# daac-tools/daachorse

Measured on AMD Instinct MI355X. Metric: haystack GB/s scanned (find_overlapping_iter(..).count(), 100k-pattern bytewise automaton), higher is better.
Workload: dtype u8/u32 integer

## Files before the change

### daachorse_amd/csrc/device_tables.hpp

```cpp
#pragma once

#include <hip/hip_runtime.h>

#include <cstdint>

#include "../../include/daachorse_amd.h"
#include "gram4_mph.hpp"

namespace daac {

struct TierDev {
    const void *rows;
    const uint32_t *bcmap;
    const uint32_t *bfail;
    const uint2 *ssum;
    const uint8_t *cls;
    const uint4 *grec;
    const uint32_t *sopos;
    const uint32_t *outputs;
    const uint32_t *ohash;
    uint32_t C, NA, NB, N;
    uint32_t off_bcmap, off_bfail, off_ssum, off_cls, lds_bytes;
    uint32_t row32, root_flag;
};

struct DArrayDev {
    const uint2 *hot;
    const uint32_t *fail;
    const uint32_t *fail_plain;
    const uint4 *rec;
    const uint4 *root_chain;
    const uint4 *root;
    const uint2 *osum;
    const uint32_t *outputs;
    const uint32_t *ohash;
    uint32_t n, root_flag, leftmost;
};

struct CharDev {
    const uint4 *states;
    const uint32_t *fail_plain;
    const uint32_t *table;
    const uint2 *osum;
    const uint32_t *outputs;
    const uint32_t *ohash;
    uint32_t table_len, n, root_flag, leftmost;
    uint32_t map_in_lds;
    uint32_t map_lo;
    const uint2 *root_row;
    uint32_t alphabet;
    uint32_t row_in_lds;
    const uint4 *wstates;
    uint32_t obits, fbits;
};

struct ScanArgs {
    const uint8_t *hay;
    uint64_t begin;
    uint64_t len;
    uint64_t seg_bytes;
    uint64_t nseg;
    uint32_t halo;
    unsigned long long *result;
    unsigned long long *seg_counts;
    daac_match *out;
    uint64_t total_len;
    unsigned long long *flags;
};

struct ScanArgs;
struct ChainArgs;

struct ChainArgs {
    const unsigned long long *x_spec;
    const unsigned long long *x_prev;
    unsigned long long *x_out;
    unsigned int *flags;
    uint4 *tally_spec;
    uint4 *tally_delta;
    uint64_t cap;
};

struct GramDev {
    const uint32_t *cls32;
    const uint16_t *cid;
    const uint2 *combo;
    const uint32_t *bbits;
    const uint8_t *brank;
    const uint32_t *bsuper;
    const uint4 *drec;
    const uint2 *dhit;
    const uint4 *dhit4;
    const uint32_t *cfirst;
    uint32_t off_cid, off_combo, off_bbits, off_brank, off_bsuper, off_scratch, lds_bytes;
    uint32_t K, C, CC, CCC;
    uint32_t level_start, unused_byte, has_short;
    uint32_t rank_in_lds;
    uint32_t n_deep;
};

struct GramArgs {
    const uint8_t *hay_al;
    uint32_t lead;
    uint64_t vlen;
    uint64_t region_bytes;
    uint64_t nregions;
    unsigned long long *result;
    uint2 *wq;
    uint32_t wq_slab;
    uint32_t ppl;
    uint32_t dense;
    const uint32_t *sel;
    uint32_t sel_want;
};

hipError_t launch_gram_scan(const GramDev &dev, const GramArgs &a, uint32_t blocks, uint32_t threads, hipStream_t stream);

constexpr uint32_t kGram2OffH = 512;
struct Gram2Dev {
    const uint8_t *cls;
    const uint32_t *m;
    const void *sdir;
    const uint16_t *rfull;
    const uint16_t *cid4;
    const uint32_t *hsum;
    const uint4 *drec;
    const uint2 *dhit;
    const uint4 *dhit4;
    const uint32_t *cfirst;
    uint32_t m_bytes, s_bytes, cid_bytes, h_bytes;
    uint32_t off_m_count, off_s_count, off_ring_count, lds_count;
    uint32_t rfull_bytes, off_ring_rfull, lds_rfull, rfull_ok;
    uint32_t off_m_exact, off_s_exact, off_cid, off_ring_exact, lds_exact;
    uint32_t K, C, s16, unused_byte, n_deep, exact_ok;
    uint32_t xlane_dpp;
};
uint32_t gram2_lds_bytes(const Gram2Dev &dev, bool exact);

struct Gram2WDev {
    const uint8_t *cls;
    const unsigned long long *m;
    const uint32_t *sdir;
    const uint16_t *cid4;
    const uint32_t *hsum;
    const uint4 *drec;
    const uint4 *dhit;
    uint32_t m_bytes, s_bytes, cid_bytes, h_bytes;
    uint32_t off_m_count, off_s_count, off_ring_count, lds_count;
    uint32_t off_m_exact, off_s_exact, off_cid, off_ring_exact, lds_exact;
    uint32_t C, unused_byte, n_deep, exact_ok;
};
hipError_t launch_gram2w_scan(const Gram2WDev &dev, const GramArgs &a, bool exact, uint32_t blocks, hipStream_t stream);

constexpr uint32_t kGram2OffM = 512;
struct Gram2EmitDev {
    const uint8_t *cls;
    const uint32_t *me;
    const void *sdir;
    const uint32_t *v1, *v2;
    const uint32_t *v3;
    const uint4 *erec;
    const uint2 *ehit;
    const uint4 *ehit4;
    const uint32_t *dupo, *dupv;
    uint32_t level_start;
    const uint32_t *cfirst;
    uint32_t m_bytes, s_bytes, v1_bytes, v2_bytes;
    uint32_t off_s, off_v1, off_v2, off_ring, off_wave, lds_bytes;
    uint32_t K, C, s16, unused_byte;
    const uint32_t *v3c;
    uint32_t v3c_bytes, v3c_dir, v3c_val;
};
hipError_t launch_gram2_scan(const Gram2Dev &dev, const GramArgs &a, bool exact, uint32_t blocks, uint32_t threads, hipStream_t stream);

struct Gram3Lds {
    uint32_t off_s;
    uint32_t off_wave;
    uint32_t wave_stride;
    uint32_t lds_bytes, threads, rfull;
};

constexpr uint32_t kGram4EndsBitDev = 30;
struct Gram4Dev {
    const uint8_t *cls;
    const uint32_t *m;
    const uint16_t *rfull;
    const void *sdir;
    const uint2 *dhit_c;
    const uint4 *dhit_t;
    const uint4 *drec_c;
    const uint4 *drec_t;
    const uint32_t *bloom;
    uint32_t bloom_words;
    const uint8_t *mph_disp;
    const uint2 *dhit_h;
    G4Mph mph;
    uint32_t mph_bytes;
    uint32_t m_bytes, rfull_bytes, s_bytes;
    uint32_t K, C, s16, arith, lo, unused_byte, n_deep;
};
struct Gram4Lds {
    uint32_t off_wave;
    uint32_t wave_stride;
    uint32_t off_cls;
    uint32_t off_s;
    uint32_t off_m;
    uint32_t s_bytes;
    uint32_t lds_bytes, threads;
    uint32_t arith;
    uint32_t dir;
    uint32_t filter;
    uint32_t off_b;
    uint32_t s_bytes_f;
    uint32_t mph;
};
uint32_t gram4_filter_room(uint32_t m_bytes, uint32_t sdir_bytes, bool arith, uint32_t lds_limit);
bool gram4_plan(const Gram4Dev &dev, uint32_t ppl, uint32_t waves, bool rfull, bool want_arith, bool want_filter, uint32_t lds_limit, Gram4Lds &L);
hipError_t launch_gram4_scan(const Gram4Dev &dev, const GramArgs &a, const Gram4Lds &L, uint32_t blocks, hipStream_t stream);

constexpr uint32_t kEmit3Tile = 1024;
constexpr uint32_t kEmit3Chunk = 1024;
constexpr uint32_t kEmit3MaxExtrasAtPosition = 15;
constexpr uint32_t kEmit3MaxExtras = 64;
constexpr uint32_t kEmit3Stage = 960;
constexpr uint32_t kEmit3ExpandWave = (kEmit3Stage + 64) * 8 + 2048 + 256 + 1024 + kEmit3MaxExtras * 16 + 16;
constexpr uint32_t kEmit3ExpandWave16 = (kEmit3Stage + 64) * 2 + 1040 + 2048 + 256 + 1024 + kEmit3MaxExtras * 16 + 16;
struct Emit3Args {
    const uint8_t *hay_al;
    uint32_t lead;
    uint32_t vlen;
    uint32_t emit_from;
    uint8_t *ann;
    uint32_t *tile_short;
    uint32_t *tile_deep;
    uint32_t tile0;
    uint4 *recs;
    uint32_t *chunk_fill;
    uint32_t *chunk_next;
    uint32_t chunk_cap;
    uint2 *wq;
    uint32_t wq_slab;
    uint32_t region_bytes;
    uint32_t nregions;
    unsigned int *fail;
};
struct Expand3Args {
    const uint8_t *ann;
    uint32_t ntiles;
    const unsigned long long *tile_off;
    const unsigned long long *bin_off;
    const uint4 *binned;
    void *out;
    unsigned long long pos_base;
    uint32_t off_wave;
    uint32_t has_len1;
    uint32_t v3_in_lds;
    unsigned int *fail;
    uint32_t vlen, emit_from;
};
bool emit3_plan(const Gram2EmitDev &dev, uint32_t waves, uint32_t lds_limit, Gram3Lds &L);
hipError_t launch_emit3_detect(const Gram2EmitDev &dev, const Emit3Args &a, const Gram3Lds &L, uint32_t blocks, hipStream_t stream);
hipError_t launch_emit3_combine(const uint32_t *tile_short, const uint32_t *tile_deep, unsigned long long *total, unsigned long long *deep, uint64_t n,
                                hipStream_t stream);
hipError_t launch_emit3_bin(const uint4 *recs, const uint32_t *chunk_fill, const uint32_t *chunk_next, uint32_t chunk_cap, const unsigned long long *bin_off,
                            uint32_t *cursor, uint4 *binned, uint32_t n1k, unsigned long long rec_limit, uint32_t blocks, hipStream_t stream);
hipError_t launch_emit3_expand(const Gram2EmitDev &dev, const Expand3Args &a, bool f16, uint32_t blocks, hipStream_t stream);
hipError_t launch_emit3_expand_raw(const Gram2EmitDev &dev, const Expand3Args &a, bool f16, uint32_t blocks, hipStream_t stream);
uint32_t emit3_expand_lds_bytes(const Gram2EmitDev &dev, uint32_t waves, bool f16, bool v3_in_lds);

constexpr uint32_t kFind3Tile = 2048;
constexpr uint32_t kFind3Deep = 255;
constexpr uint32_t kLeft3Wave = 2080 + 4096 + 1024 + 256 + 288;
constexpr uint32_t kFind3Wave = 2064 + 4096 + 1024 + 256;
struct Find3Dev {
    const uint32_t *h1, *h2;
    const uint32_t *h3c;
    uint32_t h1_bytes, h2_bytes, h3c_bytes, h3c_dir, h3c_val, C;
};
struct Find3Args {
    const uint8_t *ann;
    uint32_t ntiles;
    uint32_t n1k;
    const unsigned long long *bin_off;
    const uint4 *binned;
    const uint32_t *entry_in;
    uint32_t *exit_out;
    uint32_t force_pos;
    unsigned long long pos_base;
    uint32_t off_wave;
    uint32_t count_only;
    unsigned long long *result;
    unsigned long long *tile_cnt;
    const unsigned long long *tile_off;
    void *out;
    uint32_t f16;
    uint32_t first_start;
    uint32_t last_start;
    uint32_t *last_sel;
    unsigned int *flag;
    const uint32_t *ctl;
    uint32_t chunk_cap;
    unsigned long long rec_limit;
};
__device__ __forceinline__ bool find3_detect_usable(const Find3Args &a) {
    return a.ctl[0] <= a.chunk_cap && a.ctl[1] == 0u && a.bin_off[a.n1k] <= a.rec_limit;
}
uint32_t find3_lds_bytes(const Find3Dev &dev, bool tally);
hipError_t launch_find3_select(const Find3Dev &dev, const Find3Args &a, bool has_len1, bool tally, uint32_t blocks, hipStream_t stream);
hipError_t launch_find3_emit(const Find3Dev &dev, const Find3Args &a, bool has_len1, uint32_t blocks, hipStream_t stream);
hipError_t launch_left3_emit(const Find3Dev &dev, const Find3Args &a, bool has_len1, uint32_t blocks, hipStream_t stream);
hipError_t launch_find3_tail(const Find3Args &a, bool has_len1, uint32_t blocks, hipStream_t stream);
uint32_t left3_lds_bytes(const Find3Dev &dev, bool tally);
hipError_t launch_left3_tail(const Find3Args &a, bool has_len1, uint32_t blocks, hipStream_t stream);
hipError_t launch_left3_select(const Find3Dev &dev, const Find3Args &a, bool has_len1, bool tally, uint32_t blocks, hipStream_t stream);

struct PfxDev {
    const uint32_t *bloom;
    const uint16_t *cnt1;
    const uint16_t *disp;
    const uint4 *slots;
    const uint2 *wrec;
    const uint4 *slots_x;
    const uint4 *wrec_x;
    const uint32_t *hs1;
    const uint4 *slots_e;
    uint32_t G, has_len1, bloom_words, buckets, n_slots, seed;
    uint32_t bloom_bytes, disp_bytes;
    uint32_t off_disp, off_cnt1, off_wave, wave_stride, lds_bytes, threads;
    uint32_t n_keys;
};
bool pfx_plan(PfxDev &d, uint32_t lds_limit);
hipError_t launch_pfx_scan(const PfxDev &dev, const GramArgs &a, bool exact, uint32_t blocks, hipStream_t stream);
hipError_t launch_pfx_probe(const PfxDev &dev, const uint8_t *hay, uint64_t len, unsigned int *out, hipStream_t stream);
struct Emit3Args;
hipError_t launch_pfx_emit_detect(const PfxDev &dev, const Emit3Args &a, uint32_t blocks, hipStream_t stream);

hipError_t launch_overlap_count(const DArrayDev &dev, const ScanArgs &a, bool heads, uint32_t blocks, hipStream_t stream);
hipError_t launch_char_overlap_count(const CharDev &dev, const ScanArgs &a, bool heads, uint32_t blocks, hipStream_t stream);
hipError_t launch_tier_scan(const TierDev &dev, const ScanArgs &a, int mode, bool heads, uint32_t blocks, uint32_t threads,
                            hipStream_t stream);
hipError_t launch_darray_scan(const DArrayDev &dev, const ScanArgs &a, int mode, bool heads, uint32_t blocks, uint32_t threads,
                              hipStream_t stream);
hipError_t launch_restart_scan(const DArrayDev &dev, const ScanArgs &a, int kmode, bool leftmost, unsigned long long *next_begin,
                               uint32_t blocks, uint32_t threads, hipStream_t stream);
hipError_t launch_char_scan(const CharDev &dev, const ScanArgs &a, int mode, bool heads, uint32_t blocks, uint32_t threads,
                            hipStream_t stream);
hipError_t launch_char_restart_scan(const CharDev &dev, const ScanArgs &a, int kmode, bool leftmost, unsigned long long *next_begin,
                                    uint32_t blocks, uint32_t threads, hipStream_t stream);
hipError_t launch_chain(const DArrayDev &dev, const ScanArgs &a, const ChainArgs &c, int pass, int kmode, bool leftmost,
                        unsigned long long *next_begin, uint32_t blocks, hipStream_t stream);
hipError_t launch_char_chain(const CharDev &dev, const ScanArgs &a, const ChainArgs &c, int pass, int kmode, bool leftmost,
                             unsigned long long *next_begin, uint32_t blocks, hipStream_t stream);
hipError_t launch_exclusive_scan(unsigned long long *v, uint64_t n, unsigned long long *total, unsigned long long *scratch, hipStream_t stream);
inline uint64_t exclusive_scan_scratch(uint64_t n) { return n / 2048 + 2; }

}
```

### daachorse_amd/csrc/gram4_kernels.hip

```cpp
#include <hip/hip_runtime.h>

#include <algorithm>
#include <cstdint>
#include <utility>

#include "device_tables.hpp"
#include "gram4_filter.hpp"

namespace daac {

namespace {

typedef uint32_t g4_u32x4_t __attribute__((ext_vector_type(4)));
constexpr uint32_t kList4 = 256;
constexpr uint32_t kProbePercent4 = 3;
typedef __attribute__((address_space(3))) const uint32_t lds4_cu32;
typedef __attribute__((address_space(3))) uint32_t lds4_u32;
typedef __attribute__((address_space(3))) const uint16_t lds4_cu16;
typedef __attribute__((address_space(3))) uint16_t lds4_u16;
typedef __attribute__((address_space(3))) const uint8_t lds4_cu8;
typedef __attribute__((address_space(3))) g4_u32x4_t lds4_u32x4;

__device__ __forceinline__ uint32_t pin4(uint32_t x) {
    asm("" : "+v"(x));
    return x;
}
__device__ __forceinline__ uint32_t mad24(uint32_t a, uint32_t b, uint32_t c) {
    uint32_t d;
    asm("v_mad_u32_u24 %0, %1, %2, %3" : "=v"(d) : "v"(a), "s"(b), "v"(c));
    return d;
}
__device__ __forceinline__ uint32_t wave_shr1_4(uint32_t v, uint32_t lane0) {
    uint32_t d = lane0;
    asm volatile("s_nop 1\nv_mov_b32_dpp %0, %1 wave_shr:1 row_mask:0xf bank_mask:0xf" : "+v"(d) : "v"(v));
    return d;
}
__device__ __forceinline__ uint32_t g4_wave_scan(uint32_t v) {
    v += static_cast<uint32_t>(__builtin_amdgcn_update_dpp(0, static_cast<int>(v), 0x111, 0xf, 0xf, false));
    v += static_cast<uint32_t>(__builtin_amdgcn_update_dpp(0, static_cast<int>(v), 0x112, 0xf, 0xf, false));
    v += static_cast<uint32_t>(__builtin_amdgcn_update_dpp(0, static_cast<int>(v), 0x114, 0xf, 0xf, false));
    v += static_cast<uint32_t>(__builtin_amdgcn_update_dpp(0, static_cast<int>(v), 0x118, 0xf, 0xf, false));
    v += static_cast<uint32_t>(__builtin_amdgcn_update_dpp(0, static_cast<int>(v), 0x142, 0xa, 0xf, false));
    v += static_cast<uint32_t>(__builtin_amdgcn_update_dpp(0, static_cast<int>(v), 0x143, 0xc, 0xf, false));
    return v;
}
template <typename F, int... I>
__device__ __forceinline__ void g4_turns(F &&f, std::integer_sequence<int, I...>) {
    (void)(... && f(std::integral_constant<int, I>{}));
}
__device__ __forceinline__ unsigned long long g4_wave_sum(unsigned long long v) {
#pragma unroll
    for (int off = 32; off > 0; off >>= 1) v += __shfl_down(v, off, 64);
    return v;
}
__device__ __forceinline__ void g4_copy(void *dst, const void *src, uint32_t bytes) {
    const uint4 *s = reinterpret_cast<const uint4 *>(src);
    uint4 *d = reinterpret_cast<uint4 *>(dst);
    for (uint32_t i = threadIdx.x; i < bytes / 16; i += blockDim.x) d[i] = s[i];
}
__device__ __forceinline__ void g4_reduce(unsigned long long cnt, unsigned long long *scratch, unsigned long long *result) {
    const unsigned long long c = g4_wave_sum(cnt);
    __syncthreads();
    const int wave = threadIdx.x >> 6, lane = threadIdx.x & 63;
    if (lane == 0) scratch[wave] = c;
    __syncthreads();
    if (threadIdx.x == 0) {
        unsigned long long r0 = 0;
        for (int w = 0; w < static_cast<int>((blockDim.x + 63) >> 6); ++w) r0 += scratch[w];
        if (r0) atomicAdd(result, r0);
    }
}

}

template <int K, int Q, bool ARITH, int DIR, bool TAIL, bool FILT, bool MPH = false>
__device__ __forceinline__ void gram4_body(const Gram4Dev &g, const GramArgs &a, const Gram4Lds &L, char *smem) {
    static_assert(!(FILT && TAIL), "the filter runs in front of the plain records");
    static_assert(!(FILT && DIR == 0), "the filter's Bloom array lies where the per-word directory would");
    static_assert(!MPH || FILT, "the perfect hash serves the survivors of the filter");
    constexpr int P = 16 * Q;
    constexpr int GS = 8;
    constexpr uint32_t SB = 64u * P;
    constexpr uint32_t SLOT = SB + 32u;
    const uint32_t offM = L.off_m, offS = L.off_s, offC = L.off_cls;
    const uint32_t lo = g.lo, OTH = g.C - 1u, C = g.C;
    auto cls_of = [&](uint32_t byte) -> uint32_t {
        if (ARITH) {
            const uint32_t u = byte - lo;
            return u < OTH ? u : OTH;
        }
        return *reinterpret_cast<lds4_cu8 *>(static_cast<uintptr_t>(offC + byte));
    };
    auto lds_u32 = [&](uint32_t addr) -> uint32_t { return *reinterpret_cast<lds4_cu32 *>(static_cast<uintptr_t>(addr)); };
    auto below = [&](uint32_t k) -> uint32_t { return (1u << k) - 1u; };

    const uint32_t lane = threadIdx.x & 63;
    const uint32_t lane_off = pin4(lane * (16u * Q));
    const uint32_t wave_in_wg = __builtin_amdgcn_readfirstlane(threadIdx.x >> 6);
    const uint32_t C4 = C * 4u, CC4 = C * C * 4u;
    const uint32_t ub4 = g.unused_byte * 0x01010101u;
    const uint8_t *__restrict__ hay = a.hay_al;
    const uint64_t nwaves = static_cast<uint64_t>(gridDim.x) * (blockDim.x >> 6);
    const uint32_t tb = L.off_wave + wave_in_wg * L.wave_stride;
    const uint32_t listb = wave_in_wg * (kList4 * 2u);
    const uint64_t slab_index = (static_cast<uint64_t>(blockIdx.x) * (blockDim.x >> 6) + wave_in_wg) * a.wq_slab;
    uint4 *__restrict__ slab4 = reinterpret_cast<uint4 *>(a.wq) + slab_index;
    uint32_t wq_n = 0, slab_hi = 0;
    uint64_t epoch_base = 0;
    const uint32_t drain_early = wave_in_wg * 64u;

    unsigned long long tot_cnt = 0;
    uint32_t cnt32 = 0;

    auto load_chunk = [&](uint64_t v) -> uint4 {
        if (v >= a.vlen) return uint4{ub4, ub4, ub4, ub4};
        const g4_u32x4_t q = __builtin_nontemporal_load(reinterpret_cast<const g4_u32x4_t *>(hay + v));
        uint4 r{q.x, q.y, q.z, q.w};
        if (v < a.lead || v + 16 > a.vlen) {
            uint32_t w[4] = {r.x, r.y, r.z, r.w};
            for (int b = 0; b < 16; ++b) {
                const uint64_t p = v + b;
                if (p < a.lead || p >= a.vlen) w[b >> 2] = (w[b >> 2] & ~(0xffu << (8 * (b & 3)))) | (g.unused_byte << (8 * (b & 3)));
            }
            r = uint4{w[0], w[1], w[2], w[3]};
        }
        return r;
    };
    auto raw_at = [&](uint64_t p) -> uint32_t { return (p >= a.lead && p < a.vlen) ? hay[p] : g.unused_byte; };
    auto read_ahead = [&](uint64_t v) -> unsigned long long {
        unsigned long long x;
        if (v >= a.lead && v + 8 <= a.vlen) {
            __builtin_memcpy(&x, hay + v, 8);
        } else {
            x = 0;
            for (int b = 7; b >= 0; --b) x = (x << 8) | ((v + b >= a.lead && v + b < a.vlen) ? hay[v + b] : g.unused_byte);
        }
        return x;
    };
    auto tail_count = [&](const uint4 &rr, unsigned long long text) -> uint32_t {
        const uint32_t edges = rr.x & 15u;
        const unsigned long long path = (static_cast<unsigned long long>(rr.w) << 32) | rr.z;
        const unsigned long long diff = path ^ text;
        uint32_t same = diff ? static_cast<uint32_t>(__builtin_ctzll(diff)) >> 3 : 8u;
        same = same < edges ? same : edges;
        return __popc((rr.x >> 4) & ((2u << same) - 1u) & 0x1ffu);
    };
    auto drain = [&]() {
        const uint4 *__restrict__ recs = TAIL ? g.drec_t : g.drec_c;
        uint32_t n_in = wq_n;
        bool raw = !TAIL;
        while (n_in != 0) {
            uint32_t n_out = 0;
            for (uint32_t base = 0; base < n_in; base += 64u) {
                const uint32_t i = base + lane;
                const bool live = i < n_in;
                uint4 e = uint4{0u, 0u, 0u, 0u};
                if (live) e = slab4[i];
                uint32_t state, n_ahead;
                unsigned long long ah;
                if (raw) {
                    const uint32_t k1 = cls_of(e.w & 0xffu);
                    state = e.z + __popc(e.y & below(k1));
                    ah = e.w >> 8;
                    n_ahead = 3;
                } else {
                    state = e.y & 0x07ffffffu;
                    ah = (static_cast<unsigned long long>(e.w & 0xffffffu) << 32) | e.z;
                    n_ahead = e.w >> 24;
                }
                uint4 rr = uint4{0u, 0u, 0u, 0u};
                if (live) rr = recs[state];
                const uint64_t vn = epoch_base + e.x + 2;
                bool cont = false;
                uint32_t next_state = 0;
                if (rr.x >> 31) {
                    if (n_ahead < (rr.x & 15u)) ah = read_ahead(vn);
                    cnt32 += tail_count(rr, ah);
                } else {
                    if (live && n_ahead == 0u) { ah = read_ahead(vn); n_ahead = 8; }
                    const uint32_t k = cls_of(static_cast<uint32_t>(ah) & 0xffu);
                    cnt32 += rr.z;
                    cont = ((rr.x >> k) & 1u) != 0;
                    next_state = rr.y + __popc(rr.x & below(k));
                }
                const unsigned long long m = __ballot(cont);
                if (m != 0) {
                    if (cont) {
                        const uint32_t at = n_out + __builtin_amdgcn_mbcnt_hi(static_cast<uint32_t>(m >> 32), __builtin_amdgcn_mbcnt_lo(static_cast<uint32_t>(m), 0));
                        ah >>= 8;
                        slab4[at] = uint4{e.x + 1u, next_state, static_cast<uint32_t>(ah), static_cast<uint32_t>(ah >> 32) | ((n_ahead - 1u) << 24)};
                    }
                    n_out += static_cast<uint32_t>(__popcll(m));
                }
            }
            n_in = n_out;
            raw = false;
        }
        wq_n = 0;
    };

    uint32_t q_head = 0, q_tail = 0;
    uint32_t posbias = 0;
    uint32_t st_n = 0;
    uint32_t pend_lo = 0;
    uint4 pend = uint4{0u, 0u, 0u, 0u};
    uint32_t pend_pos = 0;
    uint32_t pend_t0 = 0, pend_t1 = 0;
    bool pend_valid = false;
    uint4 p2 = uint4{0u, 0u, 0u, 0u};
    uint32_t p2_pos = 0, p2_state = 0;
    uint32_t p2_t0 = 0, p2_t1 = 0;
    bool p2_live = false, p2_any = false;
    uint32_t sb_n = 0;
    uint32_t sb_pos = 0, sb_lo = 0, sb_t0 = 0;
    uint32_t fp_pos = 0, fp_t0 = 0;
    const uint32_t offB = L.off_b, bloomW = g.bloom_words;
    auto push_walker = [&](bool go, const uint4 &entry) {
        const unsigned long long m = __ballot(go);
        if (m != 0) {
            if (go) {
                const uint32_t at = wq_n + __builtin_amdgcn_mbcnt_hi(static_cast<uint32_t>(m >> 32), __builtin_amdgcn_mbcnt_lo(static_cast<uint32_t>(m), 0));
                slab4[at] = entry;
            }
            wq_n += __popcll(m);
        }
    };
    auto finish_second = [&]() {
        if (!TAIL || !p2_any) return;
        p2_any = false;
        const uint4 r = p2;
        bool again = false;
        uint32_t st_k = 0, pos = p2_pos, t0 = p2_t0, t1n = (p2_t1 & 0xffffffu) | (7u << 24);
        if (p2_live) {
            if (r.x >> 31) {
                if ((r.x & 15u) <= 7u) cnt32 += tail_count(r, (static_cast<unsigned long long>(p2_t1) << 32) | p2_t0);
                else { again = true; st_k = p2_state; }
            } else {
                cnt32 += r.z;
                const uint32_t k = p2_state >> 27;
                if ((r.x >> k) & 1u) {
                    again = true;
                    const uint32_t k3 = cls_of((p2_t0 >> 8) & 0xffu);
                    st_k = (r.y + __popc(r.x & below(k))) | (k3 << 27);
                    pos = p2_pos + 1u;
                    t0 = __builtin_amdgcn_alignbyte(p2_t1, p2_t0, 1u);
                    t1n = ((p2_t1 >> 8) & 0xffffu) | (6u << 24);
                }
            }
        }
        p2_live = false;
        push_walker(again, uint4{pos, st_k, t0, t1n});
    };
    auto consume_pending = [&]() {
        finish_second();
        if (!pend_valid) return;
        pend_valid = false;
        const uint4 r = pend;
        if (FILT) {
            const uint32_t k1 = cls_of(fp_t0 & 0xffu);
            cnt32 += (r.x >> kGram4EndsBitDev) & 1u;
            push_walker(__builtin_amdgcn_ubfe(r.x, k1, 1) != 0, uint4{fp_pos, r.x, r.y, fp_t0});
            return;
        }
        const uint32_t k1 = cls_of(pend_t0 & 0xffu);
        if (!TAIL) {
            cnt32 += (r.x >> kGram4EndsBitDev) & 1u;
            push_walker(__builtin_amdgcn_ubfe(r.x, k1, 1) != 0, uint4{pend_pos, r.x, r.y, pend_t0});
            return;
        }
        bool go;
        if (r.x >> 31) {
            cnt32 += tail_count(r, (static_cast<unsigned long long>(pend_t1) << 32) | pend_t0);
            go = false;
        } else {
            cnt32 += (r.x >> kGram4EndsBitDev) & 1u;
            go = ((r.x >> k1) & 1u) != 0;
        }
        p2 = uint4{0u, 0u, 0u, 0u};
        p2_live = go;
        p2_any = __ballot(go) != 0;
        if (go) {
            const uint32_t child = r.y + __popc(r.x & below(k1));
            const uint32_t k2 = cls_of((pend_t0 >> 8) & 0xffu);
            p2 = g.drec_t[child];
            p2_pos = pend_pos;
            p2_state = child | (k2 << 27);
            p2_t0 = __builtin_amdgcn_alignbyte(pend_t1, pend_t0, 1u);
            p2_t1 = pend_t1 >> 8;
        }
    };
    auto derive = [&](uint32_t first, uint32_t cnt) {
        if (lane - first < cnt) {
            const uint32_t e = tb + *reinterpret_cast<lds4_cu16 *>(static_cast<uintptr_t>(listb + ((q_head + lane - first) << 1)));
            pend_pos = e + posbias;
            const uint32_t t3 = e - 3u;
            const uint32_t a0 = t3 & ~3u, sh = t3 & 3u;
            const uint32_t d0 = lds_u32(a0), d1 = lds_u32(a0 + 4u), d2 = lds_u32(a0 + 8u);
            pend_lo = __builtin_amdgcn_alignbyte(d1, d0, sh);
            pend_t0 = __builtin_amdgcn_alignbyte(d2, d1, sh);
            if (TAIL) {
                const uint32_t d3 = lds_u32(a0 + 12u);
                pend_t1 = __builtin_amdgcn_alignbyte(d3, d2, sh);
            }
        }
        q_head += cnt;
    };
    const uint32_t lo_idx = K == 3 ? lo * (C * C + C + 1u) : lo * (C + 1u);
    auto rank_and_ask = [&](uint32_t x_lo) {
        uint32_t idx, d;
        if (ARITH) {
            idx = mad24((x_lo >> 8) & 0xffu, C, ((x_lo >> 16) & 0xffu) - lo_idx);
            if (K == 3) idx = mad24(x_lo & 0xffu, C * C, idx);
            d = (x_lo >> 24) - lo;
        } else {
            const uint32_t c1 = cls_of((x_lo >> 8) & 0xffu), c2 = cls_of((x_lo >> 16) & 0xffu);
            d = cls_of(x_lo >> 24);
            idx = __umul24(c1, C) + c2;
            if (K == 3) idx = __umul24(cls_of(x_lo & 0xffu), C * C) + idx;
        }
        const uint32_t am = (idx << 2) + offM;
        const uint32_t own = lds_u32(am);
        uint32_t rank;
        if (DIR == 0) {
            const uint32_t base = *reinterpret_cast<lds4_cu16 *>(static_cast<uintptr_t>((idx << 1) + offS));
            rank = base + __popc(own & below(d));
        } else {
            const uint32_t grp = am & ~15u;
            const uint32_t qx = lds_u32(grp), qy = lds_u32(grp + 4u), qz = lds_u32(grp + 8u);
            const uint32_t gi = pin4(idx >> 2);
            const uint32_t base = DIR == 1 ? *reinterpret_cast<lds4_cu16 *>(static_cast<uintptr_t>((gi << 1) + offS))
                                           : *reinterpret_cast<lds4_cu32 *>(static_cast<uintptr_t>((gi << 2) + offS));
            const uint32_t mx = static_cast<uint32_t>(__builtin_amdgcn_sbfe(static_cast<int>(0xEEEEEEEEu), idx, 1u));
            const uint32_t my = static_cast<uint32_t>(__builtin_amdgcn_sbfe(static_cast<int>(0xCCCCCCCCu), idx, 1u));
            const uint32_t mz = static_cast<uint32_t>(__builtin_amdgcn_sbfe(static_cast<int>(0x88888888u), idx, 1u));
            uint32_t under = __popc(own & below(d));
            under += __popc(qx & mx & 0x3fffffffu);
            under += __popc(qy & my & 0x3fffffffu);
            under += __popc(qz & mz & 0x3fffffffu);
            rank = base + under;
        }
        if (TAIL) {
            pend = g.dhit_t[rank];
        } else {
            const uint2 h = g.dhit_c[rank];
            pend = uint4{h.x, h.y, 0u, 0u};
        }
    };
    const G4Mph mph = g.mph;
    auto hash_and_ask = [&](uint32_t x_lo) {
        const uint32_t x = K == 3 ? x_lo : x_lo >> 8;
        const uint32_t h = g4f_h(x);
        const uint32_t d = *reinterpret_cast<lds4_cu8 *>(static_cast<uintptr_t>(offS + g4m_bucket(h, mph)));
        const uint2 r = g.dhit_h[g4m_slot(h, g4m_f(x, mph), d, mph)];
        pend = uint4{r.x, r.y, 0u, 0u};
    };
    auto survivors_ask = [&](uint32_t n) {
        consume_pending();
        pend = uint4{0u, 0u, 0u, 0u};
        if (lane < n) { if constexpr (MPH) hash_and_ask(sb_lo); else rank_and_ask(sb_lo); }
        fp_pos = sb_pos;
        fp_t0 = lane < n ? sb_t0 : 0u;
        pend_valid = true;
    };
    auto process_batch = [&](uint32_t n) {
        __builtin_amdgcn_s_setprio(2);
        if (FILT) {
            derive(st_n, n - st_n);
            st_n = 0;
            const G4Probe pr = g4f_probe(K == 3 ? pend_lo : pend_lo >> 8, pend_t0 & 0xffu, bloomW);
            const uint32_t fw = lds_u32(offB + (pr.word << 2));
            const bool pass = lane < n && ((pr.go & ~fw) == 0u || (pr.ends & ~fw) == 0u);
            const unsigned long long pm = __builtin_amdgcn_ballot_w64(pass);
            if (pm != 0) {
                const uint32_t s = static_cast<uint32_t>(__popcll(pm));
                const uint32_t r = __builtin_amdgcn_mbcnt_hi(static_cast<uint32_t>(pm >> 32), __builtin_amdgcn_mbcnt_lo(static_cast<uint32_t>(pm), 0));
                uint32_t t;
                asm("v_cndmask_b32_e64 %0, 63, %1, %2" : "=v"(t) : "v"(r), "s"(pm));
                const uint32_t tgt = ((t + sb_n) << 2) & 0xfcu;
                const uint32_t r_pos = static_cast<uint32_t>(__builtin_amdgcn_ds_permute(static_cast<int>(tgt), static_cast<int>(pend_pos)));
                const uint32_t r_lo = static_cast<uint32_t>(__builtin_amdgcn_ds_permute(static_cast<int>(tgt), static_cast<int>(pend_lo)));
                const uint32_t r_t0 = static_cast<uint32_t>(__builtin_amdgcn_ds_permute(static_cast<int>(tgt), static_cast<int>(pend_t0)));
                const bool mine = lane - sb_n < s;
                sb_pos = mine ? r_pos : sb_pos;
                sb_lo = mine ? r_lo : sb_lo;
                sb_t0 = mine ? r_t0 : sb_t0;
                if (sb_n + s >= 64u) {
                    survivors_ask(64u);
                    sb_pos = r_pos; sb_lo = r_lo; sb_t0 = r_t0;
                    sb_n = sb_n + s - 64u;
                } else {
                    sb_n += s;
                }
            }
            return;
        }
        consume_pending();
        derive(st_n, n - st_n);
        st_n = 0;
        pend = uint4{0u, 0u, 0u, 0u};
        if (lane < n) {
            rank_and_ask(pend_lo);
        } else {
            pend_t0 = 0;
            pend_t1 = 0;
        }
        pend_valid = true;
    };

    uint64_t region = static_cast<uint64_t>(blockIdx.x) * (blockDim.x >> 6) + wave_in_wg;
    while (region < a.nregions) {
      slab_hi = static_cast<uint32_t>((region * a.region_bytes) >> 31);
      epoch_base = static_cast<uint64_t>(slab_hi) << 31;
      for (; region < a.nregions && static_cast<uint32_t>((region * a.region_bytes) >> 31) == slab_hi; region += nwaves) {
        const uint64_t rbase = region * a.region_bytes;
        const uint64_t rend = rbase + a.region_bytes < a.vlen ? rbase + a.region_bytes : a.vlen;
        uint32_t carry = 0, tail4 = 0;
#pragma unroll
        for (int i = 0; i < K; ++i) carry |= (rbase >= static_cast<uint64_t>(K - i) ? cls_of(raw_at(rbase - (K - i))) : OTH) << (8 * i);
#pragma unroll
        for (int i = 0; i < 4; ++i) tail4 |= (rbase >= static_cast<uint64_t>(4 - i) ? raw_at(rbase - (4 - i)) : static_cast<uint32_t>(g.unused_byte)) << (8 * i);
        tail4 = __builtin_amdgcn_readfirstlane(tail4);
        carry = __builtin_amdgcn_readfirstlane(carry);
        uint32_t mcarry;
        {
            uint32_t x = (((carry >> (8 * (K - 1))) & 0xffu) << 2) + offM;
            x += __umul24((carry >> (8 * (K - 2))) & 0xffu, C4);
            if (K == 3) x += __umul24(carry & 0xffu, CC4);
            mcarry = __builtin_amdgcn_readfirstlane(lds_u32(x));
        }

        const uint32_t rlen = static_cast<uint32_t>(rend - rbase);
        const uint32_t fast_lo = rbase < 16u ? SB : 0u;
        const uint32_t fast_hi = rlen & ~(SB - 1u);
        auto fetch = [&](uint32_t off, uint4 (&out)[Q]) {
            if (off >= fast_lo && off < fast_hi) {
                const uint8_t *__restrict__ base = hay + rbase + off;
                uint32_t voff = lane_off;
                asm volatile("" : "+v"(voff));
#pragma unroll
                for (int q = 0; q < Q; ++q) {
                    const g4_u32x4_t t = __builtin_nontemporal_load(reinterpret_cast<const g4_u32x4_t *>(base + voff + 16u * q));
                    out[q] = uint4{t.x, t.y, t.z, t.w};
                }
                return;
            }
            const uint64_t s0 = rbase + off;
#pragma unroll
            for (int q = 0; q < Q; ++q) out[q] = uint4{ub4, ub4, ub4, ub4};
            if (off < rlen) {
#pragma unroll
                for (int q = 0; q < Q; ++q) out[q] = load_chunk(s0 + lane * P + 16u * q);
            } else if (lane == 0 && off < rlen + SB) {
                out[0] = load_chunk(s0);
            }
        };
        uint4 pf0[Q], pf1[Q];
        fetch(0u, pf0);
        fetch(SB, pf1);
        const uint32_t rbias = static_cast<uint32_t>(rbase - epoch_base) - (tb + 16u);

        for (uint32_t off = 0; off < rlen; off += SB) {
            if (wq_n + 64u * P + 128u + drain_early > a.wq_slab) drain();
            uint4 cur[Q];
#pragma unroll
            for (int q = 0; q < Q; ++q) { cur[q] = pf0[q]; pf0[q] = pf1[q]; }
            consume_pending();
            __builtin_amdgcn_s_setprio(0);
            fetch(off + 2u * SB, pf1);

            if (q_tail != q_head) {
                const uint32_t n_left = q_tail - q_head;
                derive(st_n, n_left);
                st_n += n_left;
            }
            q_head = q_tail = 0;
            const uint32_t slot = tb;
            const uint32_t my_text = slot + 16u + lane * P;
            posbias = rbias + off;
#pragma unroll
            for (int q = 0; q < Q; ++q)
                *reinterpret_cast<lds4_u32x4 *>(static_cast<uintptr_t>(my_text + 16u * q)) = g4_u32x4_t{cur[q].x, cur[q].y, cur[q].z, cur[q].w};
            if (lane == 0) {
                *reinterpret_cast<lds4_u32 *>(static_cast<uintptr_t>(slot + 12u)) = tail4;
                *reinterpret_cast<lds4_u32x4 *>(static_cast<uintptr_t>(slot + 16u + SB)) = g4_u32x4_t{pf0[0].x, pf0[0].y, pf0[0].z, pf0[0].w};
            }
            tail4 = __builtin_amdgcn_readlane(cur[Q - 1].w, 63);

            uint32_t kx[K + P];
#pragma unroll
            for (int q = 0; q < Q; ++q) {
                const uint32_t w[4] = {cur[q].x, cur[q].y, cur[q].z, cur[q].w};
#pragma unroll
                for (int b = 0; b < 16; ++b) {
                    kx[K + 16 * q + b] = pin4(cls_of((w[b >> 2] >> (8 * (b & 3))) & 0xffu));
                    __builtin_assume(kx[K + 16 * q + b] < 32u);
                }
            }
            uint32_t pk = 0;
#pragma unroll
            for (int i = 0; i < K; ++i) pk |= kx[P + i] << (8 * i);
            const uint32_t left = wave_shr1_4(pk, carry);
            carry = __builtin_amdgcn_readlane(pk, 63);
#pragma unroll
            for (int i = 0; i < K; ++i) { kx[i] = (left >> (8 * i)) & 0xffu; __builtin_assume(kx[i] < 32u); }

            uint32_t H = 0, ccnt = 0, roll = 0, mprev = 0;
#pragma unroll
            for (int grp = 0; grp < P / GS; ++grp) {
                uint32_t mw[GS];
#pragma unroll
                for (int jj = 0; jj < GS; ++jj) {
                    const int j = grp * GS + jj;
                    uint32_t x = pin4((kx[K + j] << 2) + offM);
                    x = mad24(kx[K + j - 1], C4, x);
                    if (K == 3) x = mad24(kx[K + j - 2], CC4, x);
                    mw[jj] = lds_u32(x);
                }
#pragma unroll
                for (int jj = 0; jj < GS; ++jj) {
                    const int j = grp * GS + jj;
                    roll = __builtin_amdgcn_alignbit(roll, mw[jj], 30);
                    if (j > 0) H = __builtin_amdgcn_alignbit((jj == 0 ? mprev : mw[jj - 1]) >> kx[K + j], H, 1);
                    if ((j & 15) == 15) {
                        ccnt += __popc(roll & 0x55555555u) + 2u * __popc(roll & 0xaaaaaaaau);
                        roll = 0;
                    }
                }
                mprev = mw[GS - 1];
            }
            {
                const uint32_t mleft = wave_shr1_4(mprev, mcarry);
                mcarry = __builtin_amdgcn_readlane(mprev, 63);
                H |= __builtin_amdgcn_ubfe(mleft, kx[K], 1) << (32 - P);
            }
            cnt32 += ccnt;

            const uint32_t text_adj = my_text - (32u - P) - tb;
            for (;;) {
                if (__ballot(H != 0u) == 0) break;
                const uint32_t n = __popc(H);
                const uint32_t incl = g4_wave_scan(n);
                const uint32_t tot = __builtin_amdgcn_readlane(incl, 63);
                const uint32_t first = q_tail + incl - n;
                const uint32_t room = first < kList4 ? kList4 - first : 0u;
                const uint32_t lim = n < room ? n : room;
                const uint32_t at = pin4(listb + (first << 1));
                g4_turns([&](auto tc) -> bool {
                    constexpr uint32_t t = decltype(tc)::value;
                    const bool w = t < lim;
                    if (__ballot(w) == 0) return false;
                    if (w) {
                        *reinterpret_cast<lds4_u16 *>(static_cast<uintptr_t>(at + 2u * t)) = static_cast<uint16_t>(text_adj + __builtin_ctz(H));
                        H &= H - 1u;
                    }
                    return true;
                }, std::make_integer_sequence<int, P>{});
                const uint32_t in = std::min(tot, kList4 - q_tail);
                q_tail += in;
                while (st_n + q_tail - q_head >= 64u) process_batch(64u);
                if (in == tot) break;
                const uint32_t n_left = q_tail - q_head;
                if (lane < n_left) {
                    const uint16_t v = *reinterpret_cast<lds4_cu16 *>(static_cast<uintptr_t>(listb + ((q_head + lane) << 1)));
                    *reinterpret_cast<lds4_u16 *>(static_cast<uintptr_t>(listb + (lane << 1))) = v;
                }
                q_head = 0;
                q_tail = n_left;
            }
        }
        tot_cnt += cnt32;
        cnt32 = 0;
      }
      if (st_n + q_tail - q_head != 0) process_batch(st_n + q_tail - q_head);
      if (FILT && sb_n != 0) { survivors_ask(sb_n); sb_n = 0; }
      consume_pending();
      finish_second();
      drain();
      tot_cnt += cnt32;
      cnt32 = 0;
    }
    g4_reduce(tot_cnt, reinterpret_cast<unsigned long long *>(smem), a.result);
}

template <int K, int Q, bool ARITH, int DIR, int TPB, bool FILT, bool MPH = false>
__global__ __launch_bounds__(TPB) void gram4_kernel(const Gram4Dev g, const GramArgs a, const Gram4Lds L) {
    extern __shared__ __attribute__((aligned(16))) char smem[];
    constexpr int DIRC = DIR == 0 ? 1 : DIR;
    if (!ARITH) g4_copy(smem + L.off_cls, g.cls, 256);
    g4_copy(smem + L.off_m, g.m, g.m_bytes);
    uint32_t *votes = reinterpret_cast<uint32_t *>(smem + L.off_wave);
    if (threadIdx.x == 0) *votes = 0;
    __syncthreads();
    if (__builtin_amdgcn_groupstaticsize() != 0) __builtin_trap();
    bool tail = a.sel_want == 1u;
    if (a.sel_want == 2u) {
        const uint64_t span = a.vlen > a.lead + 16 ? a.vlen - a.lead - 8 : 0;
        bool go = false;
        if (span != 0) {
            unsigned long long h = (static_cast<unsigned long long>(threadIdx.x) + 1) * 0x9E3779B97F4A7C15ull;
            h ^= h >> 29;
            const uint64_t p = a.lead + 3 + (h % (span - 3));
            const uint8_t *t = a.hay_al + p;
            const uint32_t OTH = g.C - 1u;
            auto cl = [&](uint32_t b) -> uint32_t {
                if (ARITH) { const uint32_t u = b - g.lo; return u < OTH ? u : OTH; }
                return reinterpret_cast<const uint8_t *>(smem + L.off_cls)[b];
            };
            const uint32_t *m = reinterpret_cast<const uint32_t *>(smem + L.off_m);
            const uint32_t c0 = cl(t[-3]), c1 = cl(t[-2]), c2 = cl(t[-1]), d = cl(t[0]), k1 = cl(t[1]);
            const uint32_t ctx = K == 3 ? (c0 * g.C + c1) * g.C + c2 : c1 * g.C + c2;
            const uint32_t w = m[ctx];
            if ((w >> d) & 1u & (d < OTH ? 1u : 0u)) {
                uint32_t rank = __popc(w & ((1u << d) - 1u));
                for (uint32_t j = ctx & ~3u; j < ctx; ++j) rank += __popc(m[j] & 0x3fffffffu);
                rank += g.s16 ? reinterpret_cast<const uint16_t *>(g.sdir)[ctx >> 2] : reinterpret_cast<const uint32_t *>(g.sdir)[ctx >> 2];
                const uint2 r = g.dhit_c[rank];
                go = ((r.x >> k1) & 1u) != 0;
            }
        }
        const unsigned long long bm = __ballot(go);
        if ((threadIdx.x & 63) == 0 && bm != 0) atomicAdd(votes, static_cast<uint32_t>(__popcll(bm)));
        __syncthreads();
        tail = *votes * 100u > static_cast<uint32_t>(TPB) * kProbePercent4;
        __syncthreads();
    }
    if (FILT && !tail) {
        g4_copy(smem + L.off_s, MPH ? static_cast<const void *>(g.mph_disp) : g.sdir, L.s_bytes_f);
        g4_copy(smem + L.off_b, g.bloom, g.bloom_words * 4u);
    } else {
        g4_copy(smem + L.off_s, DIR == 0 ? static_cast<const void *>(g.rfull) : g.sdir, L.s_bytes);
    }
    __syncthreads();
    if (tail) gram4_body<K, Q, ARITH, DIR, true, false>(g, a, L, smem);
    else if constexpr (FILT) gram4_body<K, Q, ARITH, DIRC, false, true, MPH>(g, a, L, smem);
    else gram4_body<K, Q, ARITH, DIR, false, false>(g, a, L, smem);
}

template <int K, int Q, bool ARITH, int DIR, int TPB, bool FILT, bool MPH = false>
static hipError_t launch4_inst(const Gram4Dev &dev, const GramArgs &a, const Gram4Lds &L, uint32_t blocks, hipStream_t stream) {
    const hipError_t e = hipFuncSetAttribute(reinterpret_cast<const void *>(gram4_kernel<K, Q, ARITH, DIR, TPB, FILT, MPH>),
                                             hipFuncAttributeMaxDynamicSharedMemorySize, static_cast<int>(L.lds_bytes));
    if (e != hipSuccess) return e;
    hipLaunchKernelGGL((gram4_kernel<K, Q, ARITH, DIR, TPB, FILT, MPH>), dim3(blocks), dim3(TPB), L.lds_bytes, stream, dev, a, L);
    return hipGetLastError();
}
template <int K, int Q, int TPB, bool ARITH>
static hipError_t launch4_d(const Gram4Dev &dev, const GramArgs &a, const Gram4Lds &L, uint32_t blocks, hipStream_t stream) {
    if (L.filter && L.mph) {
        if (L.dir == 0) return launch4_inst<K, Q, ARITH, 0, TPB, true, true>(dev, a, L, blocks, stream);
        if (L.dir == 1) return launch4_inst<K, Q, ARITH, 1, TPB, true, true>(dev, a, L, blocks, stream);
        return launch4_inst<K, Q, ARITH, 2, TPB, true, true>(dev, a, L, blocks, stream);
    }
    if (L.filter) {
        if (L.dir == 0) return launch4_inst<K, Q, ARITH, 0, TPB, true>(dev, a, L, blocks, stream);
        if (L.dir == 1) return launch4_inst<K, Q, ARITH, 1, TPB, true>(dev, a, L, blocks, stream);
        return launch4_inst<K, Q, ARITH, 2, TPB, true>(dev, a, L, blocks, stream);
    }
    if (L.dir == 0) return launch4_inst<K, Q, ARITH, 0, TPB, false>(dev, a, L, blocks, stream);
    if (L.dir == 1) return launch4_inst<K, Q, ARITH, 1, TPB, false>(dev, a, L, blocks, stream);
    return launch4_inst<K, Q, ARITH, 2, TPB, false>(dev, a, L, blocks, stream);
}
template <int K, int Q, int TPB>
static hipError_t launch4_k(const Gram4Dev &dev, const GramArgs &a, const Gram4Lds &L, uint32_t blocks, hipStream_t stream) {
    return L.arith ? launch4_d<K, Q, TPB, true>(dev, a, L, blocks, stream) : launch4_d<K, Q, TPB, false>(dev, a, L, blocks, stream);
}

bool gram4_plan(const Gram4Dev &dev, uint32_t ppl, uint32_t waves, bool rfull, bool want_arith, bool want_filter, uint32_t lds_limit, Gram4Lds &L) {
    L = Gram4Lds{};
    if (rfull && dev.rfull == nullptr) return false;
    const uint32_t slot = 64u * ppl + 32u;
    L.wave_stride = slot;
    L.off_wave = waves * kList4 * 2u;
    L.threads = waves * 64u;
    L.arith = (want_arith && dev.arith) ? 1u : 0u;
    const uint32_t per_wg = L.off_wave + waves * L.wave_stride;
    L.off_cls = per_wg;
    L.off_s = per_wg + (L.arith ? 0u : 256u);
    L.dir = rfull ? 0u : (dev.s16 ? 1u : 2u);
    L.s_bytes = rfull ? dev.rfull_bytes : dev.s_bytes;
    uint32_t region = L.s_bytes;
    if (want_filter && dev.bloom != nullptr) {
        const uint32_t front = dev.mph_disp != nullptr ? dev.mph_bytes : dev.s_bytes;
        const uint32_t with = front + dev.bloom_words * 4u;
        if (L.off_s + std::max(region, with) + dev.m_bytes <= lds_limit) {
            L.filter = 1u;
            L.mph = dev.mph_disp != nullptr ? 1u : 0u;
            L.s_bytes_f = front;
            L.off_b = L.off_s + front;
            region = std::max(region, with);
        }
    }
    L.off_m = L.off_s + region;
    L.lds_bytes = L.off_m + dev.m_bytes;
    return L.lds_bytes <= lds_limit;
}
uint32_t gram4_filter_room(uint32_t m_bytes, uint32_t sdir_bytes, bool arith, uint32_t lds_limit) {
    const uint32_t fixed = 16u * kList4 * 2u + 16u * (64u * 32u + 32u) + (arith ? 0u : 256u) + sdir_bytes + m_bytes;
    return fixed < lds_limit ? (lds_limit - fixed) & ~15u : 0u;
}

hipError_t launch_gram4_scan(const Gram4Dev &dev, const GramArgs &a, const Gram4Lds &L, uint32_t blocks, hipStream_t stream) {
    if (a.ppl == 32 && L.threads == 1024)
        return dev.K == 3 ? launch4_k<3, 2, 1024>(dev, a, L, blocks, stream) : launch4_k<2, 2, 1024>(dev, a, L, blocks, stream);
    if (a.ppl == 32)
        return dev.K == 3 ? launch4_k<3, 2, 512>(dev, a, L, blocks, stream) : launch4_k<2, 2, 512>(dev, a, L, blocks, stream);
    if (L.threads == 512)
        return dev.K == 3 ? launch4_k<3, 1, 512>(dev, a, L, blocks, stream) : launch4_k<2, 1, 512>(dev, a, L, blocks, stream);
    return dev.K == 3 ? launch4_k<3, 1, 1024>(dev, a, L, blocks, stream) : launch4_k<2, 1, 1024>(dev, a, L, blocks, stream);
}

}
```

Baseline: 1702.

## Give each wave a contiguous span of regions and overlap table staging

Result: no change. 1708 (median of 6 runs) (+0.3%).

```diff
diff --git a/daachorse_amd/csrc/device_tables.hpp b/daachorse_amd/csrc/device_tables.hpp
--- a/daachorse_amd/csrc/device_tables.hpp
+++ b/daachorse_amd/csrc/device_tables.hpp
@@ -112,6 +112,7 @@
     uint32_t dense;
     const uint32_t *sel;
     uint32_t sel_want;
+    uint64_t span_regions, span_extra;
 };
 
 hipError_t launch_gram_scan(const GramDev &dev, const GramArgs &a, uint32_t blocks, uint32_t threads, hipStream_t stream);
diff --git a/daachorse_amd/csrc/gram4_kernels.hip b/daachorse_amd/csrc/gram4_kernels.hip
--- a/daachorse_amd/csrc/gram4_kernels.hip
+++ b/daachorse_amd/csrc/gram4_kernels.hip
@@ -1,6 +1,7 @@
 #include <hip/hip_runtime.h>
 
 #include <algorithm>
+#include <atomic>
 #include <cstdint>
 #include <utility>
 
@@ -13,6 +14,7 @@
 
 typedef uint32_t g4_u32x4_t __attribute__((ext_vector_type(4)));
 constexpr uint32_t kList4 = 256;
+constexpr int kMaxDevices4 = 64;
 constexpr uint32_t kProbePercent4 = 3;
 typedef __attribute__((address_space(3))) const uint32_t lds4_cu32;
 typedef __attribute__((address_space(3))) uint32_t lds4_u32;
@@ -100,7 +102,6 @@
     const uint32_t C4 = C * 4u, CC4 = C * C * 4u;
     const uint32_t ub4 = g.unused_byte * 0x01010101u;
     const uint8_t *__restrict__ hay = a.hay_al;
-    const uint64_t nwaves = static_cast<uint64_t>(gridDim.x) * (blockDim.x >> 6);
     const uint32_t tb = L.off_wave + wave_in_wg * L.wave_stride;
     const uint32_t listb = wave_in_wg * (kList4 * 2u);
     const uint64_t slab_index = (static_cast<uint64_t>(blockIdx.x) * (blockDim.x >> 6) + wave_in_wg) * a.wq_slab;
@@ -407,13 +408,20 @@
         pend_valid = true;
     };
 
-    uint64_t region = static_cast<uint64_t>(blockIdx.x) * (blockDim.x >> 6) + wave_in_wg;
-    while (region < a.nregions) {
-      slab_hi = static_cast<uint32_t>((region * a.region_bytes) >> 31);
+    const uint64_t wave_id = static_cast<uint64_t>(blockIdx.x) * (blockDim.x >> 6) + wave_in_wg;
+    const uint64_t span_first = wave_id * a.span_regions + (wave_id < a.span_extra ? wave_id : a.span_extra);
+    uint64_t pos = span_first * a.region_bytes;
+    const uint64_t span_end = (span_first + a.span_regions + (wave_id < a.span_extra ? 1u : 0u)) * a.region_bytes;
+    const uint32_t fold_bytes = static_cast<uint32_t>(a.region_bytes);
+    while (pos < span_end && pos < a.vlen) {
+      slab_hi = static_cast<uint32_t>(pos >> 31);
       epoch_base = static_cast<uint64_t>(slab_hi) << 31;
-      for (; region < a.nregions && static_cast<uint32_t>((region * a.region_bytes) >> 31) == slab_hi; region += nwaves) {
-        const uint64_t rbase = region * a.region_bytes;
-        const uint64_t rend = rbase + a.region_bytes < a.vlen ? rbase + a.region_bytes : a.vlen;
+      {
+        const uint64_t epoch_end = epoch_base + (1ull << 31);
+        const uint64_t piece_end = span_end < epoch_end ? span_end : epoch_end;
+        const uint64_t rbase = pos;
+        const uint64_t rend = piece_end < a.vlen ? piece_end : a.vlen;
+        pos = piece_end;
         uint32_t carry = 0, tail4 = 0;
 #pragma unroll
         for (int i = 0; i < K; ++i) carry |= (rbase >= static_cast<uint64_t>(K - i) ? cls_of(raw_at(rbase - (K - i))) : OTH) << (8 * i);
@@ -459,7 +467,9 @@
         fetch(SB, pf1);
         const uint32_t rbias = static_cast<uint32_t>(rbase - epoch_base) - (tb + 16u);
 
-        for (uint32_t off = 0; off < rlen; off += SB) {
+        for (uint32_t off = 0; off < rlen;) {
+          const uint32_t fold_at = rlen - off > fold_bytes ? off + fold_bytes : rlen;
+          for (; off < fold_at; off += SB) {
             if (wq_n + 64u * P + 128u + drain_early > a.wq_slab) drain();
             uint4 cur[Q];
 #pragma unroll
@@ -567,9 +577,10 @@
                 q_head = 0;
                 q_tail = n_left;
             }
-        }
-        tot_cnt += cnt32;
-        cnt32 = 0;
+          }
+          tot_cnt += cnt32;
+          cnt32 = 0;
+        }
       }
       if (st_n + q_tail - q_head != 0) process_batch(st_n + q_tail - q_head);
       if (FILT && sb_n != 0) { survivors_ask(sb_n); sb_n = 0; }
@@ -588,6 +599,11 @@
     constexpr int DIRC = DIR == 0 ? 1 : DIR;
     if (!ARITH) g4_copy(smem + L.off_cls, g.cls, 256);
     g4_copy(smem + L.off_m, g.m, g.m_bytes);
+    const bool staged_early = FILT && a.sel_want != 1u;
+    if (staged_early) {
+        g4_copy(smem + L.off_s, MPH ? static_cast<const void *>(g.mph_disp) : g.sdir, L.s_bytes_f);
+        g4_copy(smem + L.off_b, g.bloom, g.bloom_words * 4u);
+    }
     uint32_t *votes = reinterpret_cast<uint32_t *>(smem + L.off_wave);
     if (threadIdx.x == 0) *votes = 0;
     __syncthreads();
@@ -624,13 +640,10 @@
         tail = *votes * 100u > static_cast<uint32_t>(TPB) * kProbePercent4;
         __syncthreads();
     }
-    if (FILT && !tail) {
-        g4_copy(smem + L.off_s, MPH ? static_cast<const void *>(g.mph_disp) : g.sdir, L.s_bytes_f);
-        g4_copy(smem + L.off_b, g.bloom, g.bloom_words * 4u);
-    } else {
+    if (!(FILT && !tail)) {
         g4_copy(smem + L.off_s, DIR == 0 ? static_cast<const void *>(g.rfull) : g.sdir, L.s_bytes);
-    }
-    __syncthreads();
+        __syncthreads();
+    }
     if (tail) gram4_body<K, Q, ARITH, DIR, true, false>(g, a, L, smem);
     else if constexpr (FILT) gram4_body<K, Q, ARITH, DIRC, false, true, MPH>(g, a, L, smem);
     else gram4_body<K, Q, ARITH, DIR, false, false>(g, a, L, smem);
@@ -638,9 +651,17 @@
 
 template <int K, int Q, bool ARITH, int DIR, int TPB, bool FILT, bool MPH = false>
 static hipError_t launch4_inst(const Gram4Dev &dev, const GramArgs &a, const Gram4Lds &L, uint32_t blocks, hipStream_t stream) {
-    const hipError_t e = hipFuncSetAttribute(reinterpret_cast<const void *>(gram4_kernel<K, Q, ARITH, DIR, TPB, FILT, MPH>),
-                                             hipFuncAttributeMaxDynamicSharedMemorySize, static_cast<int>(L.lds_bytes));
+    static std::atomic<uint32_t> raised[kMaxDevices4];
+    int device = 0;
+    hipError_t e = hipGetDevice(&device);
     if (e != hipSuccess) return e;
+    const bool known = device >= 0 && device < kMaxDevices4;
+    if (!known || raised[device].load(std::memory_order_acquire) < L.lds_bytes) {
+        e = hipFuncSetAttribute(reinterpret_cast<const void *>(gram4_kernel<K, Q, ARITH, DIR, TPB, FILT, MPH>),
+                                hipFuncAttributeMaxDynamicSharedMemorySize, static_cast<int>(L.lds_bytes));
+        if (e != hipSuccess) return e;
+        if (known) raised[device].store(L.lds_bytes, std::memory_order_release);
+    }
     hipLaunchKernelGGL((gram4_kernel<K, Q, ARITH, DIR, TPB, FILT, MPH>), dim3(blocks), dim3(TPB), L.lds_bytes, stream, dev, a, L);
     return hipGetLastError();
 }
@@ -699,7 +720,11 @@
     return fixed < lds_limit ? (lds_limit - fixed) & ~15u : 0u;
 }
 
-hipError_t launch_gram4_scan(const Gram4Dev &dev, const GramArgs &a, const Gram4Lds &L, uint32_t blocks, hipStream_t stream) {
+hipError_t launch_gram4_scan(const Gram4Dev &dev, const GramArgs &args, const Gram4Lds &L, uint32_t blocks, hipStream_t stream) {
+    GramArgs a = args;
+    const uint64_t waves = static_cast<uint64_t>(blocks) * (L.threads / 64u);
+    a.span_regions = a.nregions / waves;
+    a.span_extra = a.nregions % waves;
     if (a.ppl == 32 && L.threads == 1024)
         return dev.K == 3 ? launch4_k<3, 2, 1024>(dev, a, L, blocks, stream) : launch4_k<2, 2, 1024>(dev, a, L, blocks, stream);
     if (a.ppl == 32)
```
